# virtuoso/clap

Measured on AMD Instinct MI355X. Metric: entity updates/sec (transform hierarchy + inverse + AABB + frustum cull + visible list), higher is better.
Workload: dtype f32; 1 GPU; BASELINE configs[1]: 1000000 entities/GPU, 125000 chains x depth 8, tiles SoA layout, all dirty, fused frustum cull + ordered visible list (303309 visible); entities_per_gpu=1000000, levels=8, particles_per_gpu=0, exchange=none

## Files before the change

clap_amd/csrc/common.h:

```cpp
#pragma once
#include <hip/hip_runtime.h>
#include <stdint.h>
#include "clapgpu.h"

#define WAVE 64

namespace clapgpu {

int hip_fail(hipError_t err, const char *what);
void set_last_error(const char *what);

#define CLAPGPU_HIP(call)                                                   \
    do {                                                                    \
        hipError_t err__ = (call);                                          \
        if (err__ != hipSuccess) return ::clapgpu::hip_fail(err__, #call);  \
    } while (0)

hipError_t launch_error();
#define CLAPGPU_LAUNCH_CHECK(name)                                          \
    do {                                                                    \
        hipError_t err__ = ::clapgpu::launch_error();                       \
        if (err__ != hipSuccess) return ::clapgpu::hip_fail(err__, name);   \
    } while (0)

static inline hipStream_t as_stream(void *s) { return reinterpret_cast<hipStream_t>(s); }

__attribute__((visibility("hidden"))) int current_device_cus(int *dev, int *n_cus);

__attribute__((visibility("hidden"))) int check_bodies(const clapgpu_bodies *b);

static inline size_t align256(size_t v) { return (v + 255) & ~(size_t)255; }

struct Carve {
    size_t at = 0;
    size_t take(size_t bytes) { const size_t was = at; at += align256(bytes); return was; }
    size_t bytes() const { return at; }
};

static inline uint32_t bits_of(uint32_t v)
{
    uint32_t b = 1;
    while (b < 32 && (v >> b)) b++;
    return b;
}

__device__ __forceinline__ int lane_id() { return threadIdx.x & (WAVE - 1); }

__device__ __forceinline__ uint32_t wave_prefix_sum(uint32_t v)
{
    const int lane = lane_id();
#pragma unroll
    for (int o = 1; o < WAVE; o <<= 1) {
        const uint32_t u = __shfl_up(v, o);
        if (lane >= o) v += u;
    }
    return v;
}

__device__ __forceinline__ void wave_lds_fence()
{
    __builtin_amdgcn_fence(__ATOMIC_RELEASE, "workgroup");
    __builtin_amdgcn_wave_barrier();
    __builtin_amdgcn_fence(__ATOMIC_ACQUIRE, "workgroup");
}

__device__ __forceinline__ void stage_mat4(float4 *tile, const float (&m)[16], int lane)
{
    const int sw = (lane >> 1) & 3;
#pragma unroll
    for (int c = 0; c < 4; c++)
        tile[lane * 4 + (c ^ sw)] = make_float4(m[4 * c], m[4 * c + 1], m[4 * c + 2], m[4 * c + 3]);
}

__device__ __forceinline__ void unstage_mat4(const float4 *tile, float4 (&v)[4], int lane)
{
#pragma unroll
    for (int k = 0; k < 4; k++) {
        const int q = k * WAVE + lane;
        const int ent = q >> 2, col = q & 3;
        v[k] = tile[ent * 4 + (col ^ ((ent >> 1) & 3))];
    }
}

#if defined(CLAPGPU_EXP_NO_INVERT) || defined(CLAPGPU_EXP_NO_AABB) || defined(CLAPGPU_PLAIN_STORES) || defined(BP_SEARCH_IN_FLIGHT)
#  ifndef CLAPGPU_EXPERIMENT
#    error "CLAPGPU_EXP_* / CLAPGPU_PLAIN_STORES / BP_SEARCH_IN_FLIGHT are experiment switches: add -DCLAPGPU_EXPERIMENT (the library then reports an experiment ABI version)"
#  endif
#endif

typedef float clapgpu_f4 __attribute__((ext_vector_type(4)));
typedef float clapgpu_f2 __attribute__((ext_vector_type(2)));
typedef float clapgpu_f3 __attribute__((ext_vector_type(3), aligned(4)));
__device__ __forceinline__ void store_stream(float4 *dst, const float4 &v)
{
#ifdef CLAPGPU_PLAIN_STORES
    *dst = v;
#else
    const clapgpu_f4 t = { v.x, v.y, v.z, v.w };
    __builtin_nontemporal_store(t, reinterpret_cast<clapgpu_f4 *>(dst));
#endif
}
#ifdef CLAPGPU_PLAIN_STORES
__device__ __forceinline__ void store_stream(clapgpu_f2 *dst, const clapgpu_f2 v) { *dst = v; }
__device__ __forceinline__ void store_stream(clapgpu_f3 *dst, const clapgpu_f3 v) { *dst = v; }
#else
__device__ __forceinline__ void store_stream(clapgpu_f2 *dst, const clapgpu_f2 v) { __builtin_nontemporal_store(v, dst); }
__device__ __forceinline__ void store_stream(clapgpu_f3 *dst, const clapgpu_f3 v) { __builtin_nontemporal_store(v, dst); }
#endif

template <bool STREAM = true>
__device__ __forceinline__ void store_mat4_rows(float *dst, const float4 (&v)[4], int lane, int nvalid)
{
    float4 *out = reinterpret_cast<float4 *>(dst);
    if (nvalid == WAVE) {
#pragma unroll
        for (int k = 0; k < 4; k++) {
            if (STREAM) store_stream(&out[k * WAVE + lane], v[k]);
            else out[k * WAVE + lane] = v[k];
        }
    } else {
#pragma unroll
        for (int k = 0; k < 4; k++) {
            const int q = k * WAVE + lane;
            if ((q >> 2) < nvalid) out[q] = v[k];
        }
    }
}

template <int ROW>
__device__ __forceinline__ void stage_rows(float *tile, const float (&v)[ROW], int lane)
{
#pragma unroll
    for (int k = 0; k < ROW; k++)
        tile[lane * ROW + k] = v[k];
}

template <int ROW>
__device__ __forceinline__ void store_rows(const float *tile, float *dst, int lane, int nvalid)
{
    const int limit = nvalid * ROW;
    constexpr int CHUNKS = (WAVE * ROW + 3) / 4;
#pragma unroll
    for (int k = 0; k < (CHUNKS + WAVE - 1) / WAVE; k++) {
        const int q = k * WAVE + lane;
        if (q < CHUNKS) {
            const int f0 = 4 * q;
            if (f0 + 4 <= limit) {
                store_stream(&reinterpret_cast<float4 *>(dst)[q], reinterpret_cast<const float4 *>(tile)[q]);
            } else {
#pragma unroll
                for (int j = 0; j < 4; j++)
                    if (f0 + j < limit) dst[f0 + j] = tile[f0 + j];
            }
        }
    }
}

__device__ __forceinline__ uint32_t wave_byte_sum(const uint8_t *bytes, uint32_t nbytes, int lane)
{
    const uint4 *p = reinterpret_cast<const uint4 *>(bytes);
    const uint32_t chunks = nbytes >> 4;
    uint32_t acc = 0;
    for (uint32_t c = lane; c < chunks; c += WAVE * 8) {
        uint4 v[8];
#pragma unroll
        for (int u = 0; u < 8; u++) {
            const uint32_t idx = c + u * WAVE;
            v[u] = idx < chunks ? p[idx] : make_uint4(0, 0, 0, 0);
        }
#pragma unroll
        for (int u = 0; u < 8; u++) {
            acc = __builtin_amdgcn_sad_u8(v[u].x, 0u, acc);
            acc = __builtin_amdgcn_sad_u8(v[u].y, 0u, acc);
            acc = __builtin_amdgcn_sad_u8(v[u].z, 0u, acc);
            acc = __builtin_amdgcn_sad_u8(v[u].w, 0u, acc);
        }
    }
#pragma unroll
    for (int off = 32; off > 0; off >>= 1)
        acc += __shfl_xor(acc, off);
    return acc;
}

}

__attribute__((visibility("hidden"))) int clapgpu_bodies_ground_apply(void *stream, const clapgpu_bodies *b, uint32_t n,
                                                                      const uint32_t *body, const double *ray_off,
                                                                      const uint8_t *grounded, uint8_t *grounded_out,
                                                                      const double *dist, const int32_t *hit, uint32_t *flags,
                                                                      const uint32_t *moved);
__attribute__((visibility("hidden"))) int clapgpu_bodies_slide_apply(void *stream, const clapgpu_bodies *b, uint32_t n,
                                                                     const uint32_t *body, uint32_t *flags, const uint32_t *moved);
__attribute__((visibility("hidden"))) int clapgpu_bodies_ground_collide_on(void *stream, struct clapgpu_bp *bp,
                                                                           const clapgpu_bodies *b, const clapgpu_geoms *statics,
                                                                           const clapgpu_trimesh *meshes, uint32_t n,
                                                                           const uint32_t *body, const double *ray_off,
                                                                           const uint8_t *grounded, uint8_t *grounded_out,
                                                                           float *normal, double *dist, int32_t *hit,
                                                                           uint32_t *flags, uint32_t *scratch, double *other,
                                                                           bool cleared);
```

clap_amd/csrc/visible.hip:

```cpp
#include <string.h>
#include <math.h>
#include "common.h"
#include "lm_dev.h"
#include "entities_row.h"
#include "entities_args.h"

namespace clapgpu {

template <class... XV>
__global__ __launch_bounds__(ENT_BLOCK)
void k_entities_cull(const uint32_t *flags, const float *aabb, uint64_t *vis_mask, uint8_t *vis_row_pop,
                     uint32_t n, lmd::FrustumK fr, XV... xv)
{
    const uint32_t i = blockIdx.x * ENT_BLOCK + threadIdx.x;
    const int lane = lane_id();
    bool base = false, vis = false;
    uint32_t fl = 0;
    float bb[6] = { 0, 0, 0, 0, 0, 0 };
    if (i < n) {
        fl = flags[i];
        base = (fl & CLAPGPU_E_ALIVE) && (fl & CLAPGPU_E_VISIBLE);
        vis = base;
        if (base && !(fl & CLAPGPU_E_SKIP_CULLING)) {
#pragma unroll
            for (int k = 0; k < 6; k++) bb[k] = aabb[6 * (size_t)i + k];
            vis = lmd::aabb_in_frustum_fast(fr, bb);
        }
    }
    if constexpr (sizeof...(XV) != 0)
        if ((i - lane) >= n) return;
    const uint64_t m = __ballot(vis);
    if (lane == 0 && (i - lane) < n) {
        vis_mask[i >> 6] = m;
        vis_row_pop[i >> 6] = (uint8_t)__popcll(m);
    }
    if constexpr (sizeof...(XV) != 0) cull_extra_views(xv..., base, fl, bb, i >> 6, lane);
}

constexpr int GROUP_WORDS = 64;

__device__ __forceinline__ uint64_t load_mask_word(const uint64_t *vis_mask, uint32_t w, uint32_t n)
{
    const uint32_t nwords = (n + 63) / 64;
    if (w >= nwords)
        return 0;
    uint64_t v = vis_mask[w];
    const uint32_t rem = n - w * 64;
    if (rem < 64)
        v &= (1ull << rem) - 1ull;
    return v;
}

__device__ __forceinline__ uint32_t wave_sum(uint32_t v)
{
#pragma unroll
    for (int off = 32; off > 0; off >>= 1)
        v += __shfl_xor(v, off);
    return v;
}

__global__ __launch_bounds__(WAVE)
void k_mask_group_count(const uint64_t *vis_mask, uint32_t n, uint32_t *group_count)
{
    const uint32_t w = blockIdx.x * GROUP_WORDS + threadIdx.x;
    const uint32_t c = wave_sum(__popcll(load_mask_word(vis_mask, w, n)));
    if (threadIdx.x == 0)
        group_count[blockIdx.x] = c;
}

__global__ __launch_bounds__(WAVE)
void k_visible_expand(const uint64_t *vis_mask, uint32_t n, const uint32_t *group_count,
                      uint32_t n_groups, uint32_t index_base, uint32_t *visible, uint32_t *count)
{
    const int lane = threadIdx.x;
    const uint32_t g = blockIdx.x;

    uint32_t pre = 0;
    for (uint32_t j = lane; j < g; j += WAVE)
        pre += group_count[j];
    pre = wave_sum(pre);

    const uint64_t word = load_mask_word(vis_mask, g * GROUP_WORDS + lane, n);
    const uint32_t cnt = __popcll(word);
    uint32_t incl = cnt;
#pragma unroll
    for (int off = 1; off < WAVE; off <<= 1) {
        uint32_t t = __shfl_up(incl, off);
        if (lane >= off) incl += t;
    }
    const uint32_t excl = incl - cnt;

    for (int k = 0; k < GROUP_WORDS; k++) {
        const uint64_t wk = __shfl(word, k);
        if (wk == 0) continue;
        const uint32_t base = pre + __shfl(excl, k);
        if ((wk >> lane) & 1ull) {
            const uint32_t rank = __popcll(wk & ((1ull << lane) - 1ull));
            visible[base + rank] = index_base + (g * GROUP_WORDS + k) * 64u + lane;
        }
    }
    if (g == n_groups - 1 && lane == WAVE - 1)
        *count = pre + incl;
}

constexpr int MAX_SEGMENTS = 64;
struct SegK { uint32_t cap_words, n_seg; uint32_t base[MAX_SEGMENTS], n_words[MAX_SEGMENTS]; };

__device__ __forceinline__ uint64_t load_seg_word(const uint64_t *mask, const SegK &sg, uint32_t w, uint32_t *id_base)
{
    const uint32_t r = w / sg.cap_words, lw = w - r * sg.cap_words;
    if (r >= sg.n_seg || lw >= sg.n_words[r]) { *id_base = 0; return 0ull; }
    *id_base = sg.base[r] + lw * 64u;
    return mask[w];
}

__global__ __launch_bounds__(WAVE)
void k_mask_group_count_seg(const uint64_t *mask, SegK sg, uint32_t *group_count)
{
    uint32_t idb;
    const uint32_t c = wave_sum(__popcll(load_seg_word(mask, sg, blockIdx.x * GROUP_WORDS + threadIdx.x, &idb)));
    if (threadIdx.x == 0)
        group_count[blockIdx.x] = c;
}

__global__ __launch_bounds__(WAVE)
void k_visible_expand_seg(const uint64_t *mask, SegK sg, const uint32_t *group_count, uint32_t n_groups, uint32_t *visible,
                          uint32_t *count)
{
    const int lane = threadIdx.x;
    const uint32_t g = blockIdx.x;
    uint32_t pre = 0;
    for (uint32_t j = lane; j < g; j += WAVE)
        pre += group_count[j];
    pre = wave_sum(pre);
    uint32_t idb;
    const uint64_t word = load_seg_word(mask, sg, g * GROUP_WORDS + lane, &idb);
    const uint32_t cnt = __popcll(word);
    uint32_t incl = cnt;
#pragma unroll
    for (int off = 1; off < WAVE; off <<= 1) {
        uint32_t t = __shfl_up(incl, off);
        if (lane >= off) incl += t;
    }
    const uint32_t excl = incl - cnt;
    for (int k = 0; k < GROUP_WORDS; k++) {
        const uint64_t wk = __shfl(word, k);
        if (wk == 0) continue;
        const uint32_t base = pre + __shfl(excl, k), ids = __shfl(idb, k);
        if ((wk >> lane) & 1ull) {
            const uint32_t rank = __popcll(wk & ((1ull << lane) - 1ull));
            visible[base + rank] = ids + lane;
        }
    }
    if (g == n_groups - 1 && lane == WAVE - 1)
        *count = pre + incl;
}

constexpr int RP_ROWS = 16;
constexpr uint32_t RP_MAX_ROWS = 1u << 16;

__device__ __forceinline__ uint32_t sum_bytes(uint32_t v, uint32_t acc)
{
    return __builtin_amdgcn_sad_u8(v, 0u, acc);
}

__global__ __launch_bounds__(ENT_BLOCK)
void k_visible_expand_rp(const uint64_t *vis_mask, const uint8_t *row_pop, uint32_t n,
                         uint32_t index_base, uint32_t *visible, uint32_t *count)
{
    const int lane = lane_id();
    const uint32_t g = blockIdx.x * (ENT_BLOCK / WAVE) + threadIdx.x / WAVE;
    const uint32_t n_rows = (n + 63) / 64;
    const uint32_t row0 = g * RP_ROWS;
    if (row0 >= n_rows)
        return;

    const uint32_t pre = wave_byte_sum(row_pop, row0, lane);

    const uint64_t word = lane < RP_ROWS ? load_mask_word(vis_mask, row0 + lane, n) : 0ull;
    const uint32_t cnt = __popcll(word);
    uint32_t incl = cnt;
#pragma unroll
    for (int off = 1; off < RP_ROWS; off <<= 1) {
        uint32_t t = __shfl_up(incl, off);
        if (lane >= off) incl += t;
    }
    const uint32_t excl = incl - cnt;
    const uint32_t lo = (uint32_t)word, hi = (uint32_t)(word >> 32);

#pragma unroll
    for (int k = 0; k < RP_ROWS; k++) {
        const uint64_t wk = (uint64_t)(uint32_t)__builtin_amdgcn_readlane(lo, k) |
                            ((uint64_t)(uint32_t)__builtin_amdgcn_readlane(hi, k) << 32);
        if (wk == 0) continue;
        const uint32_t base = pre + (uint32_t)__builtin_amdgcn_readlane(excl, k);
        if ((wk >> lane) & 1ull) {
            const uint32_t rank = __popcll(wk & ((1ull << lane) - 1ull));
            visible[base + rank] = index_base + (row0 + k) * 64u + lane;
        }
    }
    if (row0 + RP_ROWS >= n_rows && lane == RP_ROWS - 1)
        *count = pre + incl;
}

__device__ __forceinline__ float cbrtf_glibc(float x)
{
    int xe;
    const float xm = frexpf(fabsf(x), &xe);
    if (xe == 0 && (x == 0.0f || x != x || isinf(x)))
        return x + x;
    const float u = (float)(0.492659620528969547 + (0.697570460207922770 - 0.191502161678719066 * (double)xm) * (double)xm);
    const float t2 = u * u * u;
    const int r = xe % 3;
    const double f = r == -2 ? 1.0 / 1.5874010519681994748 : r == -1 ? 1.0 / 1.2599210498948731648
                   : r == 0 ? 1.0 : r == 1 ? 1.2599210498948731648 : 1.5874010519681994748;
    const float ym = (float)((double)u * ((double)t2 + 2.0 * (double)xm) / (2.0 * (double)t2 + (double)xm) * f);
    return ldexpf(x > 0.0f ? ym : -ym, xe / 3);
}

struct LodK {
    float cx, cy, cz;
    const float *aabb, *center;
    const float4 *pos_scale;
    const int32_t *model;
    const float4 *model_table;
    const int32_t *force_lod;
    int32_t *cur_lod;
    uint32_t n_models;
};

__device__ __forceinline__ int32_t lod_pick(const LodK &k, uint32_t i)
{
    int32_t lod = k.cur_lod[i];
    const int32_t forced = k.force_lod ? k.force_lod[i] : -1;
    if (forced >= 0) {
        lod = forced;
    } else {
        const float *b = k.aabb + 6 * (size_t)i;
        const bool inside = k.cx >= b[0] && k.cx <= b[3] && k.cy >= b[1] && k.cy <= b[4] && k.cz >= b[2] && k.cz <= b[5];
        if (!inside) {
            const float *c = k.center + 3 * (size_t)i;
            const float dx = c[0] - k.cx, dy = c[1] - k.cy, dz = c[2] - k.cz;
            float dd = 0.f;
            dd += dx * dx;
            dd += dy * dy;
            dd += dz * dz;
            const int32_t mraw = k.model[i];
            const int32_t mi = (uint32_t)mraw < k.n_models ? mraw : 0;
            const float4 lo = k.model_table[2 * mi], hi = k.model_table[2 * mi + 1];
            const float s = k.pos_scale[i].w;
            const float X = fabsf(hi.x - lo.x) * s, Y = fabsf(hi.y - lo.y) * s, Z = fabsf(hi.z - lo.z) * s;
            const float side = cbrtf_glibc(X * Y * Z);
            const float scale = (float)((double)fabsf(dd - side * side) / 3600.0);
            const uint32_t lm = __float_as_uint(hi.w);
            const int lmin = (int)(lm & 0xffu), lmax = (int)((lm >> 8) & 0xffu);
            const int req = (int)scale;
            lod = req < lmin ? lmin : (req > lmax ? lmax : req);
        }
    }
    k.cur_lod[i] = lod;
    return lod;
}

__global__ __launch_bounds__(ENT_BLOCK)
void k_entities_lod(const uint32_t *visible, const uint32_t *count, uint32_t index_base, LodK lk, int32_t *draw_lod, uint32_t n)
{
    const uint32_t total = *count < n ? *count : n;
    for (uint32_t k = blockIdx.x * ENT_BLOCK + threadIdx.x; k < total; k += gridDim.x * ENT_BLOCK) {
        const uint32_t i = visible[k] - index_base;
        if (i >= n) { draw_lod[k] = 0; continue; }
        draw_lod[k] = lod_pick(lk, i);
    }
}

}

using namespace clapgpu;

extern "C" int clapgpu_entities_cull(void *stream, const clapgpu_entities *e, const clapgpu_frustum *frustum)
{
    if (!e || !frustum || !e->flags || !e->aabb || !e->vis_mask || !e->vis_row_pop)
        return CLAPGPU_ERR_INVALID_ARGUMENTS;
    if (e->n == 0)
        return CLAPGPU_OK;
    const lmd::FrustumK fr = make_frustum_k(frustum);
    XViewsK xv;
    if (!make_xviews_k(e, false, &xv)) return CLAPGPU_ERR_INVALID_ARGUMENTS;
    const dim3 grid((e->n + ENT_BLOCK - 1) / ENT_BLOCK), block(ENT_BLOCK);
    if (xv.n)
        hipLaunchKernelGGL(k_entities_cull<XViewsK>, grid, block, 0, as_stream(stream), e->flags, e->aabb, e->vis_mask,
                           e->vis_row_pop, e->n, fr, xv);
    else
        hipLaunchKernelGGL(k_entities_cull<>, grid, block, 0, as_stream(stream), e->flags, e->aabb, e->vis_mask,
                           e->vis_row_pop, e->n, fr);
    CLAPGPU_LAUNCH_CHECK("k_entities_cull");
    return CLAPGPU_OK;
}

extern "C" size_t clapgpu_visible_scratch_bytes(uint32_t n)
{
    const uint32_t n_groups = (n + GROUP_WORDS * 64 - 1) / (GROUP_WORDS * 64);
    return (size_t)(n_groups ? n_groups : 1) * sizeof(uint32_t);
}

extern "C" int clapgpu_visible_compact(void *stream, const uint64_t *vis_mask, const uint8_t *vis_row_pop,
                                       uint32_t n, uint32_t index_base, uint32_t *visible, uint32_t *count,
                                       void *scratch)
{
    if (!count || (n && (!vis_mask || !visible)))
        return CLAPGPU_ERR_INVALID_ARGUMENTS;
    if (n == 0) {
        CLAPGPU_HIP(hipMemsetAsync(count, 0, sizeof(uint32_t), as_stream(stream)));
        return CLAPGPU_OK;
    }
    const uint32_t n_rows = (n + 63) / 64;
    if (vis_row_pop && n_rows <= RP_MAX_ROWS && aligned16(vis_row_pop)) {
        const uint32_t waves = (n_rows + RP_ROWS - 1) / RP_ROWS, per_block = ENT_BLOCK / WAVE;
        hipLaunchKernelGGL(k_visible_expand_rp, dim3((waves + per_block - 1) / per_block), dim3(ENT_BLOCK), 0,
                           as_stream(stream), vis_mask, vis_row_pop, n, index_base, visible, count);
        CLAPGPU_LAUNCH_CHECK("k_visible_expand_rp");
        return CLAPGPU_OK;
    }
    if (!scratch)
        return CLAPGPU_ERR_INVALID_ARGUMENTS;
    const uint32_t n_groups = (n + GROUP_WORDS * 64 - 1) / (GROUP_WORDS * 64);
    uint32_t *group_count = static_cast<uint32_t *>(scratch);
    hipLaunchKernelGGL(k_mask_group_count, dim3(n_groups), dim3(WAVE), 0, as_stream(stream), vis_mask, n, group_count);
    CLAPGPU_LAUNCH_CHECK("k_mask_group_count");
    hipLaunchKernelGGL(k_visible_expand, dim3(n_groups), dim3(WAVE), 0, as_stream(stream), vis_mask, n,
                       group_count, n_groups, index_base, visible, count);
    CLAPGPU_LAUNCH_CHECK("k_visible_expand");
    return CLAPGPU_OK;
}

static int check_ranges(uint32_t n_ranges, uint32_t cap_pad, const uint32_t *base, const uint32_t *n_pad)
{
    if (!n_ranges || n_ranges > (uint32_t)MAX_SEGMENTS || !cap_pad || (cap_pad & 63u) || !base) return CLAPGPU_ERR_INVALID_ARGUMENTS;
    uint64_t end = 0;
    for (uint32_t r = 0; r < n_ranges; r++) {
        const uint32_t np = n_pad ? n_pad[r] : cap_pad;
        if ((np & 63u) || np > cap_pad || (base[r] & 63u) || base[r] < end) return CLAPGPU_ERR_INVALID_ARGUMENTS;
        end = (uint64_t)base[r] + np;
        if (end > 0xffffffffull) return CLAPGPU_ERR_TOO_LARGE;
    }
    return CLAPGPU_OK;
}

extern "C" int clapgpu_visible_compact_ranges(void *stream, const uint64_t *gathered_mask, uint32_t n_ranges, uint32_t cap_pad,
                                              const uint32_t *base, const uint32_t *n_pad, uint32_t *visible, uint32_t *count,
                                              void *scratch)
{
    if (!gathered_mask || !visible || !count || !scratch) return CLAPGPU_ERR_INVALID_ARGUMENTS;
    int rc = check_ranges(n_ranges, cap_pad, base, n_pad);
    if (rc) return rc;
    SegK sg = {};
    sg.cap_words = cap_pad / 64; sg.n_seg = n_ranges;
    for (uint32_t r = 0; r < n_ranges; r++) { sg.base[r] = base[r]; sg.n_words[r] = (n_pad ? n_pad[r] : cap_pad) / 64; }
    const uint64_t total_words = (uint64_t)sg.cap_words * n_ranges;
    if (total_words * 64 > 0xffffffffull) return CLAPGPU_ERR_TOO_LARGE;
    const uint32_t n_groups = (uint32_t)((total_words + GROUP_WORDS - 1) / GROUP_WORDS);
    uint32_t *group_count = static_cast<uint32_t *>(scratch);
    hipLaunchKernelGGL(k_mask_group_count_seg, dim3(n_groups), dim3(WAVE), 0, as_stream(stream), gathered_mask, sg, group_count);
    CLAPGPU_LAUNCH_CHECK("k_mask_group_count_seg");
    hipLaunchKernelGGL(k_visible_expand_seg, dim3(n_groups), dim3(WAVE), 0, as_stream(stream), gathered_mask, sg, group_count, n_groups,
                       visible, count);
    CLAPGPU_LAUNCH_CHECK("k_visible_expand_seg");
    return CLAPGPU_OK;
}

extern "C" uint32_t clapgpu_visible_expand_ranges_host(const uint64_t *gathered_mask, uint32_t n_ranges, uint32_t cap_pad,
                                                       const uint32_t *base, const uint32_t *n_pad, uint32_t *visible, uint32_t capacity)
{
    if (!gathered_mask || check_ranges(n_ranges, cap_pad, base, n_pad)) return 0;
    const uint32_t cap_words = cap_pad / 64;
    uint32_t cnt = 0;
    for (uint32_t r = 0; r < n_ranges; r++) {
        const uint32_t words = (n_pad ? n_pad[r] : cap_pad) / 64;
        for (uint32_t w = 0; w < words; w++) {
            uint64_t m = gathered_mask[(size_t)r * cap_words + w];
            while (m) {
                const uint32_t id = base[r] + w * 64u + (uint32_t)__builtin_ctzll(m);
                m &= m - 1;
                if (visible && cnt < capacity) visible[cnt] = id;
                cnt++;
            }
        }
    }
    return cnt;
}

static LodK lod_args(const clapgpu_entities *e, const float cam_pos[3], const int32_t *force_lod, int32_t *cur_lod)
{
    LodK k;
    k.cx = cam_pos[0]; k.cy = cam_pos[1]; k.cz = cam_pos[2];
    k.aabb = e->aabb; k.center = e->center;
    k.pos_scale = reinterpret_cast<const float4 *>(e->pos_scale);
    k.model = e->model;
    k.model_table = reinterpret_cast<const float4 *>(e->model_table);
    k.force_lod = force_lod; k.cur_lod = cur_lod;
    k.n_models = e->n_models ? e->n_models : 1;
    return k;
}

extern "C" int clapgpu_entities_lod(void *stream, const clapgpu_entities *e, const uint32_t *visible,
                                    const uint32_t *count, uint32_t index_base, const float cam_pos[3],
                                    const int32_t *force_lod, int32_t *cur_lod, int32_t *draw_lod)
{
    if (!e || !visible || !count || !cam_pos || !cur_lod || !draw_lod || !e->aabb || !e->center ||
        !e->pos_scale || !e->model || !e->model_table)
        return CLAPGPU_ERR_INVALID_ARGUMENTS;
    if (e->n == 0)
        return CLAPGPU_OK;
    uint32_t blocks = (e->n + ENT_BLOCK - 1) / ENT_BLOCK;
    if (blocks > 2048) blocks = 2048;
    hipLaunchKernelGGL(k_entities_lod, dim3(blocks), dim3(ENT_BLOCK), 0, as_stream(stream), visible, count, index_base,
                       lod_args(e, cam_pos, force_lod, cur_lod), draw_lod, e->n);
    CLAPGPU_LAUNCH_CHECK("k_entities_lod");
    return CLAPGPU_OK;
}

extern "C" int clapgpu_visible_compact_lod(void *stream, const clapgpu_entities *e, uint32_t index_base, const float cam_pos[3],
                                           const int32_t *force_lod, int32_t *cur_lod, uint32_t *visible, uint32_t *count,
                                           int32_t *draw_lod, void *scratch)
{
    if (!e || !count || !cam_pos || !cur_lod || !draw_lod || (e->n && (!e->vis_mask || !visible)) || !e->aabb || !e->center ||
        !e->pos_scale || !e->model || !e->model_table)
        return CLAPGPU_ERR_INVALID_ARGUMENTS;
    const uint32_t n = e->n;
    int rc = clapgpu_visible_compact(stream, e->vis_mask, e->vis_row_pop, n, index_base, visible, count, scratch);
    if (rc) return rc;
    return clapgpu_entities_lod(stream, e, visible, count, index_base, cam_pos, force_lod, cur_lod, draw_lod);
}
```

Before: 23.16 billion entity updates/s.

## Share visible-list prefix sums across block waves and batch in-flight loads

The row-pop expand kernel now splits the byte-sum over all earlier rows across the whole block instead of repeating it per wave, then combines per-wave partials and intra-block totals through shared memory. Loads are issued in fixed unrolled batches before the reduction, so more memory requests are in flight at once. The group-count expand kernels get a similar unrolled u32 prefix sum. The cost is a block barrier and a larger, templated load path. An experiment switch that makes the kernel return immediately is also added.

```diff
diff --git a/clap_amd/csrc/common.h b/clap_amd/csrc/common.h
--- a/clap_amd/csrc/common.h
+++ b/clap_amd/csrc/common.h
@@ -82,7 +82,8 @@
     }
 }
 
-#if defined(CLAPGPU_EXP_NO_INVERT) || defined(CLAPGPU_EXP_NO_AABB) || defined(CLAPGPU_PLAIN_STORES) || defined(BP_SEARCH_IN_FLIGHT)
+#if defined(CLAPGPU_EXP_NO_INVERT) || defined(CLAPGPU_EXP_NO_AABB) || defined(CLAPGPU_EXP_EXPAND_EMPTY) || defined(CLAPGPU_PLAIN_STORES) || \
+    defined(BP_SEARCH_IN_FLIGHT)
 #  ifndef CLAPGPU_EXPERIMENT
 #    error "CLAPGPU_EXP_* / CLAPGPU_PLAIN_STORES / BP_SEARCH_IN_FLIGHT are experiment switches: add -DCLAPGPU_EXPERIMENT (the library then reports an experiment ABI version)"
 #  endif
diff --git a/clap_amd/csrc/visible.hip b/clap_amd/csrc/visible.hip
--- a/clap_amd/csrc/visible.hip
+++ b/clap_amd/csrc/visible.hip
@@ -59,6 +59,24 @@
     return v;
 }
 
+constexpr int SUM_IN_FLIGHT = 8;
+__device__ __forceinline__ uint32_t wave_u32_sum(const uint32_t *v, uint32_t n, int lane)
+{
+    uint32_t acc = 0;
+    for (uint32_t c = 0; c < n; c += WAVE * SUM_IN_FLIGHT) {
+        uint32_t t[SUM_IN_FLIGHT];
+#pragma unroll
+        for (int u = 0; u < SUM_IN_FLIGHT; u++) {
+            const uint32_t idx = c + u * WAVE + lane;
+            t[u] = v[idx < n ? idx : 0u];
+        }
+#pragma unroll
+        for (int u = 0; u < SUM_IN_FLIGHT; u++)
+            acc += c + u * WAVE + lane < n ? t[u] : 0u;
+    }
+    return wave_sum(acc);
+}
+
 __global__ __launch_bounds__(WAVE)
 void k_mask_group_count(const uint64_t *vis_mask, uint32_t n, uint32_t *group_count)
 {
@@ -75,10 +93,7 @@
     const int lane = threadIdx.x;
     const uint32_t g = blockIdx.x;
 
-    uint32_t pre = 0;
-    for (uint32_t j = lane; j < g; j += WAVE)
-        pre += group_count[j];
-    pre = wave_sum(pre);
+    const uint32_t pre = wave_u32_sum(group_count, g, lane);
 
     const uint64_t word = load_mask_word(vis_mask, g * GROUP_WORDS + lane, n);
     const uint32_t cnt = __popcll(word);
@@ -129,10 +144,7 @@
 {
     const int lane = threadIdx.x;
     const uint32_t g = blockIdx.x;
-    uint32_t pre = 0;
-    for (uint32_t j = lane; j < g; j += WAVE)
-        pre += group_count[j];
-    pre = wave_sum(pre);
+    const uint32_t pre = wave_u32_sum(group_count, g, lane);
     uint32_t idb;
     const uint64_t word = load_seg_word(mask, sg, g * GROUP_WORDS + lane, &idb);
     const uint32_t cnt = __popcll(word);
@@ -164,20 +176,61 @@
     return __builtin_amdgcn_sad_u8(v, 0u, acc);
 }
 
+constexpr int RP_WAVES = ENT_BLOCK / WAVE;
+
+template <int T>
+__device__ __forceinline__ uint32_t rp_load(const uint8_t *row_pop, uint32_t chunks, const uint64_t *vis_mask, uint32_t w,
+                                            bool own, uint32_t n, uint64_t *word)
+{
+    const uint4 *p = reinterpret_cast<const uint4 *>(row_pop);
+    const uint32_t n_rows = (n + 63) / 64;
+    uint4 v[T ? T : 1];
+#pragma unroll
+    for (int u = 0; u < T; u++) {
+        const uint32_t idx = threadIdx.x + u * ENT_BLOCK;
+        v[u] = p[idx < chunks ? idx : 0u];
+    }
+    const uint64_t raw = vis_mask[own ? w : n_rows - 1];
+#pragma unroll
+    for (int u = 0; u < T; u++)
+        asm volatile("" : : "v"(v[u].x));
+    asm volatile("" : : "v"((uint32_t)raw));
+    uint32_t acc = 0;
+#pragma unroll
+    for (int u = 0; u < T; u++) {
+        const bool in = threadIdx.x + u * ENT_BLOCK < chunks;
+        acc = sum_bytes(in ? v[u].x : 0u, acc);
+        acc = sum_bytes(in ? v[u].y : 0u, acc);
+        acc = sum_bytes(in ? v[u].z : 0u, acc);
+        acc = sum_bytes(in ? v[u].w : 0u, acc);
+    }
+    const uint32_t rem = n - w * 64;
+    *word = !own ? 0ull : rem < 64 ? raw & ((1ull << rem) - 1ull) : raw;
+    return acc;
+}
+
 __global__ __launch_bounds__(ENT_BLOCK)
 void k_visible_expand_rp(const uint64_t *vis_mask, const uint8_t *row_pop, uint32_t n,
                          uint32_t index_base, uint32_t *visible, uint32_t *count)
 {
+    __shared__ uint32_t part[RP_WAVES], total[RP_WAVES];
+#ifdef CLAPGPU_EXP_EXPAND_EMPTY
+    return;
+#endif
     const int lane = lane_id();
-    const uint32_t g = blockIdx.x * (ENT_BLOCK / WAVE) + threadIdx.x / WAVE;
+    const uint32_t wave = threadIdx.x / WAVE;
     const uint32_t n_rows = (n + 63) / 64;
-    const uint32_t row0 = g * RP_ROWS;
-    if (row0 >= n_rows)
-        return;
-
-    const uint32_t pre = wave_byte_sum(row_pop, row0, lane);
-
-    const uint64_t word = lane < RP_ROWS ? load_mask_word(vis_mask, row0 + lane, n) : 0ull;
+    const uint32_t row0 = (blockIdx.x * RP_WAVES + wave) * RP_ROWS;
+    const uint32_t chunks = blockIdx.x * (RP_WAVES * RP_ROWS / 16);
+    const bool own = lane < RP_ROWS && row0 + lane < n_rows;
+
+    uint64_t word;
+    uint32_t acc;
+    if (chunks == 0) acc = rp_load<0>(row_pop, chunks, vis_mask, row0 + lane, own, n, &word);
+    else if (chunks <= 4 * ENT_BLOCK) acc = rp_load<4>(row_pop, chunks, vis_mask, row0 + lane, own, n, &word);
+    else acc = rp_load<RP_MAX_ROWS / 16 / ENT_BLOCK>(row_pop, chunks, vis_mask, row0 + lane, own, n, &word);
+    acc = wave_sum(acc);
+
     const uint32_t cnt = __popcll(word);
     uint32_t incl = cnt;
 #pragma unroll
@@ -187,6 +240,13 @@
     }
     const uint32_t excl = incl - cnt;
     const uint32_t lo = (uint32_t)word, hi = (uint32_t)(word >> 32);
+
+    if (lane == RP_ROWS - 1) { part[wave] = acc; total[wave] = incl; }
+    __syncthreads();
+    uint32_t pre = 0;
+#pragma unroll
+    for (uint32_t k = 0; k < RP_WAVES; k++)
+        pre += part[k] + (k < wave ? total[k] : 0u);
 
 #pragma unroll
     for (int k = 0; k < RP_ROWS; k++) {
@@ -199,7 +259,7 @@
             visible[base + rank] = index_base + (row0 + k) * 64u + lane;
         }
     }
-    if (row0 + RP_ROWS >= n_rows && lane == RP_ROWS - 1)
+    if (row0 < n_rows && row0 + RP_ROWS >= n_rows && lane == RP_ROWS - 1)
         *count = pre + incl;
 }
 
```

Result: faster. 23.75 billion entity updates/s (median of 6 runs) (+2.5%).
